# SonyResearch/micro_diffusion

Measured on NVIDIA H100. Metric: training images/sec (global batch 2048), higher is better.
Workload: dtype bf16

## Files before the change

### micro_diffusion_b200/csrc/attn.cu

```cuda
#include <stdlib.h>

#include <initializer_list>

#include "common.cuh"

namespace md {

constexpr int kTile = 64;

__device__ __forceinline__ void ldsm_x4(uint32_t (&r)[4], const void* p) {
  const uint32_t a = static_cast<uint32_t>(__cvta_generic_to_shared(p));
  asm volatile("ldmatrix.sync.aligned.m8n8.x4.shared.b16 {%0,%1,%2,%3}, [%4];"
               : "=r"(r[0]), "=r"(r[1]), "=r"(r[2]), "=r"(r[3])
               : "r"(a));
}
__device__ __forceinline__ void ldsm_x4_t(uint32_t (&r)[4], const void* p) {
  const uint32_t a = static_cast<uint32_t>(__cvta_generic_to_shared(p));
  asm volatile("ldmatrix.sync.aligned.m8n8.x4.trans.shared.b16 {%0,%1,%2,%3}, [%4];"
               : "=r"(r[0]), "=r"(r[1]), "=r"(r[2]), "=r"(r[3])
               : "r"(a));
}
__device__ __forceinline__ void mma16816(float (&d)[4], const uint32_t (&a)[4], uint32_t b0, uint32_t b1) {
  asm volatile(
      "mma.sync.aligned.m16n8k16.row.col.f32.bf16.bf16.f32 {%0,%1,%2,%3}, {%4,%5,%6,%7}, {%8,%9}, {%0,%1,%2,%3};"
// ... 303 lines not shown
  if constexpr (!kFragsInSmem) {
    load_a_frags<HD>(ka, sk, warp * 16, lane);
    load_a_frags<HD>(va, sv, warp * 16, lane);
  }

  float dkacc[HD / 8][4], dvacc[HD / 8][4];
#pragma unroll
  for (int i = 0; i < HD / 8; ++i)
#pragma unroll
    for (int j = 0; j < 4; ++j) dkacc[i][j] = dvacc[i][j] = 0.f;

  for (int q0 = 0, it = 0; q0 < Tq; q0 += kTile, ++it) {
    const __nv_bfloat16* sq = sqdo + (it & 1) * (2 * kTile * P);
    const __nv_bfloat16* sdo = sq + kTile * P;
    const float* slse = sstat + (it & 1) * 2 * kTile;
    const float* sdelta = slse + kTile;
    if (q0 + kTile < Tq) {
      prefetch(q0 + kTile, (it + 1) & 1);
      cp_async_wait<1>();
    } else {
      cp_async_wait<0>();
    }
    __syncthreads();
    float st[8][4], dpt[8][4];
#pragma unroll
    for (int i = 0; i < 8; ++i)
#pragma unroll
      for (int j = 0; j < 4; ++j) st[i][j] = dpt[i][j] = 0.f;
    if constexpr (kFragsInSmem) {
      mma_sa_bt<HD>(st, sk, warp * 16, sq, lane);
      mma_sa_bt<HD>(dpt, sv, warp * 16, sdo, lane);
    } else {
      mma_a_bt<HD>(st, ka, sq, lane);
      mma_a_bt<HD>(dpt, va, sdo, lane);
    }
#pragma unroll
    for (int nt = 0; nt < 8; ++nt)
#pragma unroll
      for (int j = 0; j < 4; ++j) {
        const int qc = nt * 8 + 2 * t + (j & 1);
        const float p = exp2f(st[nt][j] * scale_log2 - slse[qc]);
        st[nt][j] = p;
        dpt[nt][j] = p * (dpt[nt][j] - sdelta[qc]);
      }
    uint32_t pa[4][4];
    acc_to_afrag(pa, st);
    mma_p_m<HD>(dvacc, pa, sdo, lane);
    acc_to_afrag(pa, dpt);
    mma_p_m<HD>(dkacc, pa, sq, lane);
    __syncthreads();
  }
#pragma unroll
  for (int r = 0; r < 2; ++r) {
    const int key = k0 + warp * 16 + g + r * 8;
    if (key < Tk) {
      __nv_bfloat16* pk = dk + (b * Tk + key) * lddk + h * HD;
      __nv_bfloat16* pv = dv + (b * Tk + key) * lddv + h * HD;
#pragma unroll
      for (int i = 0; i < HD / 8; ++i) {
        *reinterpret_cast<uint32_t*>(pk + i * 8 + 2 * t) = pack2(dkacc[i][2 * r] * scale, dkacc[i][2 * r + 1] * scale);
        *reinterpret_cast<uint32_t*>(pv + i * 8 + 2 * t) = pack2(dvacc[i][2 * r], dvacc[i][2 * r + 1]);
      }
    }
  }
}

template <int HD>
__global__ void __launch_bounds__(128)
attn_bwd_dq_kernel(const __nv_bfloat16* __restrict__ dout, long long lddo, const __nv_bfloat16* __restrict__ q,
                   long long ldq, const __nv_bfloat16* __restrict__ k, long long ldk,
                   const __nv_bfloat16* __restrict__ v, long long ldv, const float* __restrict__ lse,
                   const float* __restrict__ delta, __nv_bfloat16* __restrict__ dq, long long lddq, int H, int Tq,
                   int Tk, float scale, float scale_log2) {
  constexpr int P = Smem<HD>::kPitch;
  __shared__ __align__(16) __nv_bfloat16 sq[kTile * P];
  __shared__ __align__(16) __nv_bfloat16 sdo[kTile * P];
  extern __shared__ __align__(16) unsigned char smem_dq[];
  __nv_bfloat16* skv = reinterpret_cast<__nv_bfloat16*>(smem_dq);
  const int warp = threadIdx.x >> 5, lane = threadIdx.x & 31;
  const int g = lane >> 2, t = lane & 3;
  const int h = blockIdx.y;
  const long long b = blockIdx.z;
  const int q0 = blockIdx.x * kTile;
  const __nv_bfloat16* kg = k + b * Tk * ldk;
  const __nv_bfloat16* vg = v + b * Tk * ldv;

  load_tile_async<HD>(skv, kg, ldk, 0, Tk, h * HD);
  load_tile_async<HD>(skv + kTile * P, vg, ldv, 0, Tk, h * HD);
  cp_async_commit();
  load_tile<HD>(sq, q + b * Tq * ldq, ldq, q0, Tq, h * HD);
  load_tile<HD>(sdo, dout + b * Tq * lddo, lddo, q0, Tq, h * HD);
  __syncthreads();
  uint32_t qa[HD / 16][4], doa[HD / 16][4];
  load_a_frags<HD>(qa, sq, warp * 16, lane);
  load_a_frags<HD>(doa, sdo, warp * 16, lane);
  float lrow[2], drow[2];
#pragma unroll
  for (int r = 0; r < 2; ++r) {
    const int row = q0 + warp * 16 + g + r * 8;
    lrow[r] = row < Tq ? lse[(b * H + h) * Tq + row] : INFINITY;
    drow[r] = row < Tq ? delta[(b * H + h) * Tq + row] : 0.f;
  }
  float dqacc[HD / 8][4];
#pragma unroll
  for (int i = 0; i < HD / 8; ++i)
#pragma unroll
    for (int j = 0; j < 4; ++j) dqacc[i][j] = 0.f;

  for (int k0 = 0, it = 0; k0 < Tk; k0 += kTile, ++it) {
    __nv_bfloat16* sk = skv + (it & 1) * (2 * kTile * P);
    __nv_bfloat16* sv = sk + kTile * P;
    if (k0 + kTile < Tk) {
      __nv_bfloat16* nk = skv + ((it + 1) & 1) * (2 * kTile * P);
      load_tile_async<HD>(nk, kg, ldk, k0 + kTile, Tk, h * HD);
      load_tile_async<HD>(nk + kTile * P, vg, ldv, k0 + kTile, Tk, h * HD);
      cp_async_commit();
      cp_async_wait<1>();
    } else {
      cp_async_wait<0>();
    }
    __syncthreads();
    float s[8][4], dp[8][4];
#pragma unroll
    for (int i = 0; i < 8; ++i)
#pragma unroll
      for (int j = 0; j < 4; ++j) s[i][j] = dp[i][j] = 0.f;
    mma_a_bt<HD>(s, qa, sk, lane);
    mma_a_bt<HD>(dp, doa, sv, lane);
#pragma unroll
    for (int nt = 0; nt < 8; ++nt)
#pragma unroll
      for (int j = 0; j < 4; ++j) {
        const int key = k0 + nt * 8 + 2 * t + (j & 1);
        const float p = key < Tk ? exp2f(s[nt][j] * scale_log2 - lrow[j >> 1]) : 0.f;
        s[nt][j] = p * (dp[nt][j] - drow[j >> 1]);
      }
    uint32_t pa[4][4];
    acc_to_afrag(pa, s);
    mma_p_m<HD>(dqacc, pa, sk, lane);
    __syncthreads();
  }
#pragma unroll
  for (int r = 0; r < 2; ++r) {
    const int row = q0 + warp * 16 + g + r * 8;
    if (row < Tq) {
      __nv_bfloat16* dst = dq + (b * Tq + row) * lddq + h * HD;
#pragma unroll
      for (int i = 0; i < HD / 8; ++i)
        *reinterpret_cast<uint32_t*>(dst + i * 8 + 2 * t) = pack2(dqacc[i][2 * r] * scale, dqacc[i][2 * r + 1] * scale);
    }
  }
}

template <int HD, int KT>
__global__ void __launch_bounds__(128)
attn_bwd_small_kernel(const __nv_bfloat16* __restrict__ dout, long long lddo, const __nv_bfloat16* __restrict__ q,
                      long long ldq, const __nv_bfloat16* __restrict__ k, long long ldk,
                      const __nv_bfloat16* __restrict__ v, long long ldv, const float* __restrict__ lse,
                      __nv_bfloat16* __restrict__ dq, long long lddq, __nv_bfloat16* __restrict__ dk, long long lddk,
                      __nv_bfloat16* __restrict__ dv, long long lddv, int H, int Tq, int Tk, float scale,
                      float scale_log2) {
  constexpr int P = Smem<HD>::kPitch;
  constexpr int PP = KT + 8;
  extern __shared__ __align__(16) unsigned char smem_small[];
  __nv_bfloat16* sq = reinterpret_cast<__nv_bfloat16*>(smem_small);
  __nv_bfloat16* sdo = sq + kTile * P;
  __nv_bfloat16* sk = sdo + kTile * P;
  __nv_bfloat16* sv = sk + KT * P;
  static_assert(kTile * (KT + 8) <= KT * Smem<HD>::kPitch || HD == 32, "P copy must fit in the K tile");
  __nv_bfloat16* sp = (HD == 64) ? sk : sv + KT * P;
  __nv_bfloat16* sds = (HD == 64) ? sv : sp + kTile * PP;
  const int warp = threadIdx.x >> 5, lane = threadIdx.x & 31;
  const int g = lane >> 2, t = lane & 3;
  const int h = blockIdx.x;
  const long long b = blockIdx.y;

  load_tile<HD>(sq, q + b * Tq * ldq, ldq, 0, Tq, h * HD);
  load_tile<HD>(sdo, dout + b * Tq * lddo, lddo, 0, Tq, h * HD);
  load_tile<HD, KT>(sk, k + b * Tk * ldk, ldk, 0, Tk, h * HD);
  load_tile<HD, KT>(sv, v + b * Tk * ldv, ldv, 0, Tk, h * HD);
  float lrow[2];
#pragma unroll
  for (int r = 0; r < 2; ++r) {
    const int row = warp * 16 + g + r * 8;
    lrow[r] = row < Tq ? lse[(b * H + h) * Tq + row] : INFINITY;
  }
  __syncthreads();

  uint32_t qa[HD / 16][4], doa[HD / 16][4];
  load_a_frags<HD>(qa, sq, warp * 16, lane);
  load_a_frags<HD>(doa, sdo, warp * 16, lane);
  float s[KT / 8][4], dp[KT / 8][4];
#pragma unroll
  for (int i = 0; i < KT / 8; ++i)
#pragma unroll
    for (int j = 0; j < 4; ++j) s[i][j] = dp[i][j] = 0.f;
  mma_a_bt<HD, KT>(s, qa, sk, lane);
  mma_a_bt<HD, KT>(dp, doa, sv, lane);
  float dsum[2] = {0.f, 0.f};
#pragma unroll
  for (int nt = 0; nt < KT / 8; ++nt)
#pragma unroll
    for (int j = 0; j < 4; ++j) {
      const int key = nt * 8 + 2 * t + (j & 1);
      const float p = key < Tk ? exp2f(s[nt][j] * scale_log2 - lrow[j >> 1]) : 0.f;
      s[nt][j] = p;
      dsum[j >> 1] += p * dp[nt][j];
    }
#pragma unroll
  for (int r = 0; r < 2; ++r) {
    dsum[r] += __shfl_xor_sync(0xffffffffu, dsum[r], 1);
    dsum[r] += __shfl_xor_sync(0xffffffffu, dsum[r], 2);
  }
#pragma unroll
  for (int nt = 0; nt < KT / 8; ++nt)
#pragma unroll
    for (int j = 0; j < 4; ++j) dp[nt][j] = s[nt][j] * (dp[nt][j] - dsum[j >> 1]);
  {
    uint32_t pa[KT / 16][4];
    acc_to_afrag<KT / 16>(pa, dp);
    float dqacc[HD / 8][4];
#pragma unroll
    for (int i = 0; i < HD / 8; ++i)
#pragma unroll
      for (int j = 0; j < 4; ++j) dqacc[i][j] = 0.f;
    mma_p_m<HD, KT>(dqacc, pa, sk, lane);
#pragma unroll
    for (int r = 0; r < 2; ++r) {
      const int row = warp * 16 + g + r * 8;
      if (row < Tq) {
        __nv_bfloat16* dst = dq + (b * Tq + row) * lddq + h * HD;
#pragma unroll
        for (int i = 0; i < HD / 8; ++i)
          *reinterpret_cast<uint32_t*>(dst + i * 8 + 2 * t) = pack2(dqacc[i][2 * r] * scale, dqacc[i][2 * r + 1] * scale);
      }
    }
  }
  __syncthreads();
#pragma unroll
  for (int nt = 0; nt < KT / 8; ++nt)
#pragma unroll
    for (int r = 0; r < 2; ++r) {
      const int row = warp * 16 + g + r * 8;
      *reinterpret_cast<uint32_t*>(sp + row * PP + nt * 8 + 2 * t) = pack2(s[nt][2 * r], s[nt][2 * r + 1]);
      *reinterpret_cast<uint32_t*>(sds + row * PP + nt * 8 + 2 * t) = pack2(dp[nt][2 * r], dp[nt][2 * r + 1]);
    }
  __syncthreads();
  for (int kb = warp; kb < KT / 16; kb += 4) {
    uint32_t pta[4][4], dsta[4][4];
#pragma unroll
    for (int ks = 0; ks < 4; ++ks) {
      const int mi = lane >> 3;
      const int rowq = ks * 16 + (lane & 7) + (mi >> 1) * 8;
      const int colk = kb * 16 + (mi & 1) * 8;
      ldsm_x4_t(pta[ks], sp + rowq * PP + colk);
      ldsm_x4_t(dsta[ks], sds + rowq * PP + colk);
    }
    float dvacc[HD / 8][4], dkacc[HD / 8][4];
#pragma unroll
    for (int i = 0; i < HD / 8; ++i)
#pragma unroll
      for (int j = 0; j < 4; ++j) dvacc[i][j] = dkacc[i][j] = 0.f;
    mma_p_m<HD, 64>(dvacc, pta, sdo, lane);
    mma_p_m<HD, 64>(dkacc, dsta, sq, lane);
#pragma unroll
    for (int r = 0; r < 2; ++r) {
      const int key = kb * 16 + g + r * 8;
      if (key < Tk) {
        __nv_bfloat16* pk = dk + (b * Tk + key) * lddk + h * HD;
        __nv_bfloat16* pv = dv + (b * Tk + key) * lddv + h * HD;
#pragma unroll
        for (int i = 0; i < HD / 8; ++i) {
          *reinterpret_cast<uint32_t*>(pk + i * 8 + 2 * t) = pack2(dkacc[i][2 * r] * scale, dkacc[i][2 * r + 1] * scale);
          *reinterpret_cast<uint32_t*>(pv + i * 8 + 2 * t) = pack2(dvacc[i][2 * r], dvacc[i][2 * r + 1]);
        }
      }
    }
  }
}

template <int HD, int DP>
__device__ __forceinline__ void mma_p_m_slice(float (&out)[2][4], const uint32_t (&pa)[4][4], const __nv_bfloat16* m,
                                              int lane, int dp) {
#pragma unroll
  for (int kt = 0; kt < 4; ++kt) {
    uint32_t b[4];
    const int mi = lane >> 3;
    ldsm_x4_t(b, m + (kt * 16 + (lane & 7) + (mi & 1) * 8) * Smem<HD>::kPitch + dp * 16 + (mi >> 1) * 8);
    mma16816(out[0], pa[kt], b[0], b[1]);
    mma16816(out[1], pa[kt], b[2], b[3]);
  }
}

template <int HD, int KT>
__global__ void __launch_bounds__(128)
attn_bwd_cross_kernel(const __nv_bfloat16* __restrict__ dout, long long lddo, const __nv_bfloat16* __restrict__ q,
                      long long ldq, const __nv_bfloat16* __restrict__ k, long long ldk,
                      const __nv_bfloat16* __restrict__ v, long long ldv, const float* __restrict__ lse,
                      __nv_bfloat16* __restrict__ dq, long long lddq, __nv_bfloat16* __restrict__ dk, long long lddk,
                      __nv_bfloat16* __restrict__ dv, long long lddv, int H, int Tq, int Tk, float scale,
                      float scale_log2) {
  constexpr int P = Smem<HD>::kPitch;
  constexpr int PP = KT + 8;
  constexpr bool kExtra = KT > 64;
  constexpr int kSliceWarps = HD / 16;
  extern __shared__ __align__(16) unsigned char smem_cross[];
  __nv_bfloat16* sk = reinterpret_cast<__nv_bfloat16*>(smem_cross);
  __nv_bfloat16* sv = sk + KT * P;
  __nv_bfloat16* sqdo = sv + KT * P;
  __nv_bfloat16* sp = sqdo + 4 * kTile * P;
  __nv_bfloat16* sds = sp + kTile * PP;
  const int warp = threadIdx.x >> 5, lane = threadIdx.x & 31;
  const int g = lane >> 2, t = lane & 3;
  const int h = blockIdx.x;
  const long long b = blockIdx.y;
  const __nv_bfloat16* qg = q + b * Tq * ldq;
  const __nv_bfloat16* dog = dout + b * Tq * lddo;
  const float* lseg = lse + (b * H + h) * Tq;

  auto prefetch = [&](int q0, int buf) {
    __nv_bfloat16* dst = sqdo + buf * (2 * kTile * P);
    load_tile_async<HD>(dst, qg, ldq, q0, Tq, h * HD);
    load_tile_async<HD>(dst + kTile * P, dog, lddo, q0, Tq, h * HD);
    cp_async_commit();
  };
  load_tile_async<HD, KT>(sk, k + b * Tk * ldk, ldk, 0, Tk, h * HD);
  load_tile_async<HD, KT>(sv, v + b * Tk * ldv, ldv, 0, Tk, h * HD);
  prefetch(0, 0);

  float dvacc[HD / 8][4], dkacc[HD / 8][4];
  float dvx[2][4], dkx[2][4];
#pragma unroll
  for (int i = 0; i < HD / 8; ++i)
#pragma unroll
    for (int j = 0; j < 4; ++j) dvacc[i][j] = dkacc[i][j] = 0.f;
#pragma unroll
  for (int i = 0; i < 2; ++i)
#pragma unroll
    for (int j = 0; j < 4; ++j) dvx[i][j] = dkx[i][j] = 0.f;

  for (int q0 = 0, it = 0; q0 < Tq; q0 += kTile, ++it) {
    const __nv_bfloat16* sq = sqdo + (it & 1) * (2 * kTile * P);
    const __nv_bfloat16* sdo = sq + kTile * P;
    float lrow[2];
#pragma unroll
    for (int r = 0; r < 2; ++r) {
      const int row = q0 + warp * 16 + g + r * 8;
      lrow[r] = row < Tq ? lseg[row] : INFINITY;
    }
    if (q0 + kTile < Tq) {
      prefetch(q0 + kTile, (it + 1) & 1);
      cp_async_wait<1>();
    } else {
      cp_async_wait<0>();
    }
    __syncthreads();

    uint32_t qa[HD / 16][4], doa[HD / 16][4];
    load_a_frags<HD>(qa, sq, warp * 16, lane);
    load_a_frags<HD>(doa, sdo, warp * 16, lane);
    float s[KT / 8][4], dp[KT / 8][4];
#pragma unroll
    for (int i = 0; i < KT / 8; ++i)
#pragma unroll
      for (int j = 0; j < 4; ++j) s[i][j] = dp[i][j] = 0.f;
    mma_a_bt<HD, KT>(s, qa, sk, lane);
    mma_a_bt<HD, KT>(dp, doa, sv, lane);
    float dsum[2] = {0.f, 0.f};
#pragma unroll
    for (int nt = 0; nt < KT / 8; ++nt)
#pragma unroll
      for (int j = 0; j < 4; ++j) {
        const int key = nt * 8 + 2 * t + (j & 1);
        const float pr = key < Tk ? exp2f(s[nt][j] * scale_log2 - lrow[j >> 1]) : 0.f;
        s[nt][j] = pr;
        dsum[j >> 1] += pr * dp[nt][j];
      }
#pragma unroll
    for (int r = 0; r < 2; ++r) {
      dsum[r] += __shfl_xor_sync(0xffffffffu, dsum[r], 1);
      dsum[r] += __shfl_xor_sync(0xffffffffu, dsum[r], 2);
    }
#pragma unroll
    for (int nt = 0; nt < KT / 8; ++nt)
#pragma unroll
      for (int j = 0; j < 4; ++j) dp[nt][j] = s[nt][j] * (dp[nt][j] - dsum[j >> 1]);
    {
      uint32_t pa[KT / 16][4];
      acc_to_afrag<KT / 16>(pa, dp);
      float dqacc[HD / 8][4];
#pragma unroll
      for (int i = 0; i < HD / 8; ++i)
#pragma unroll
        for (int j = 0; j < 4; ++j) dqacc[i][j] = 0.f;
      mma_p_m<HD, KT>(dqacc, pa, sk, lane);
#pragma unroll
      for (int r = 0; r < 2; ++r) {
        const int row = q0 + warp * 16 + g + r * 8;
        if (row < Tq) {
          __nv_bfloat16* dst = dq + (b * Tq + row) * lddq + h * HD;
#pragma unroll
          for (int i = 0; i < HD / 8; ++i)
            *reinterpret_cast<uint32_t*>(dst + i * 8 + 2 * t) = pack2(dqacc[i][2 * r] * scale, dqacc[i][2 * r + 1] * scale);
        }
      }
    }
#pragma unroll
    for (int nt = 0; nt < KT / 8; ++nt)
#pragma unroll
      for (int r = 0; r < 2; ++r) {
        const int row = warp * 16 + g + r * 8;
        *reinterpret_cast<uint32_t*>(sp + row * PP + nt * 8 + 2 * t) = pack2(s[nt][2 * r], s[nt][2 * r + 1]);
        *reinterpret_cast<uint32_t*>(sds + row * PP + nt * 8 + 2 * t) = pack2(dp[nt][2 * r], dp[nt][2 * r + 1]);
      }
    __syncthreads();
    {
      uint32_t pta[4][4], dsta[4][4];
#pragma unroll
      for (int ks = 0; ks < 4; ++ks) {
        const int mi = lane >> 3;
        const int rowq = ks * 16 + (lane & 7) + (mi >> 1) * 8;
        const int colk = warp * 16 + (mi & 1) * 8;
        ldsm_x4_t(pta[ks], sp + rowq * PP + colk);
        ldsm_x4_t(dsta[ks], sds + rowq * PP + colk);
      }
      mma_p_m<HD, 64>(dvacc, pta, sdo, lane);
      mma_p_m<HD, 64>(dkacc, dsta, sq, lane);
      if (kExtra && warp < kSliceWarps) {
#pragma unroll
        for (int ks = 0; ks < 4; ++ks) {
          const int mi = lane >> 3;
          const int rowq = ks * 16 + (lane & 7) + (mi >> 1) * 8;
          const int colk = 64 + (mi & 1) * 8;
          ldsm_x4_t(pta[ks], sp + rowq * PP + colk);
          ldsm_x4_t(dsta[ks], sds + rowq * PP + colk);
        }
        mma_p_m_slice<HD, 0>(dvx, pta, sdo, lane, warp);
        mma_p_m_slice<HD, 0>(dkx, dsta, sq, lane, warp);
      }
    }
    __syncthreads();
  }

#pragma unroll
  for (int r = 0; r < 2; ++r) {
// ... 230 lines not shown
```

### micro_diffusion_b200/csrc/attn_wgmma.cu

```cuda
#include <cuda.h>

#include "common.cuh"
#include "ptx.cuh"
#include "tensormap.cuh"

namespace md {
namespace attn_wg {

constexpr int kHd = 64;
constexpr int kQ = 64;
constexpr int kMaxKeys = 256;
constexpr int kOffK = kQ * kHd * 2;
constexpr int kOffV = kOffK + kMaxKeys * kHd * 2;
constexpr int kOffBar = kOffV + kMaxKeys * kHd * 2;
constexpr int kSmemBytes = kOffBar + 64 + 1024;

__device__ __forceinline__ float ex2_approx(float x) {
  float y;
  asm("ex2.approx.ftz.f32 %0, %1;" : "=f"(y) : "f"(x));
  return y;
}
__device__ __forceinline__ uint32_t pack2(float a, float b) {
  __nv_bfloat162 v = __floats2bfloat162_rn(a, b);
  return *reinterpret_cast<uint32_t*>(&v);
// ... 194 lines not shown
    }
    wgmma_commit();
    wgmma_wait<0>();
    wgmma_fence_operands(s);

    float mx[2] = {-INFINITY, -INFINITY};
#pragma unroll
    for (int j = 0; j < 8; ++j)
#pragma unroll
      for (int i = 0; i < 2; ++i)
#pragma unroll
        for (int e = 0; e < 2; ++e) {
          float& v = s[4 * j + 2 * i + e];
          if (c * 64 + 8 * j + cq + e >= Tk) v = -INFINITY;
          mx[i] = fmaxf(mx[i], v);
        }
    float corr[2];
#pragma unroll
    for (int i = 0; i < 2; ++i) {
      mx[i] = fmaxf(mx[i], __shfl_xor_sync(0xffffffffu, mx[i], 1));
      mx[i] = fmaxf(mx[i], __shfl_xor_sync(0xffffffffu, mx[i], 2));
      const float mn = fmaxf(m2[i], mx[i] * sl2);
      corr[i] = ex2_approx(m2[i] - mn);
      m2[i] = mn;
      l[i] *= corr[i];
    }
#pragma unroll
    for (int j = 0; j < 8; ++j)
#pragma unroll
      for (int i = 0; i < 2; ++i)
#pragma unroll
        for (int e = 0; e < 2; ++e) {
          float& v = s[4 * j + 2 * i + e];
          v = ex2_approx(fmaf(v, sl2, -m2[i]));
          l[i] += v;
        }
#pragma unroll
    for (int x = 0; x < 2; ++x)
#pragma unroll
      for (int j = 0; j < 8; ++j)
#pragma unroll
        for (int i = 0; i < 2; ++i) {
          oacc[x][4 * j + 2 * i] *= corr[i];
          oacc[x][4 * j + 2 * i + 1] *= corr[i];
        }

    uint32_t pa[4][4];
#pragma unroll
    for (int t = 0; t < 4; ++t)
#pragma unroll
      for (int r = 0; r < 4; ++r) pa[t][r] = pack2(s[8 * t + 2 * r], s[8 * t + 2 * r + 1]);
    const uint64_t dv0 = wgmma_smem_desc(smem_u32(st + 2 * kBox), 64 * 128, 1024);
    const uint64_t dv1 = wgmma_smem_desc(smem_u32(st + 3 * kBox), 64 * 128, 1024);
    wgmma_fence();
#pragma unroll
    for (int t = 0; t < 4; ++t) {
      wgmma_m64n64k16_rs<1>(oacc[0], pa[t], dv0 + static_cast<uint64_t>(t * 128), 1u);
      wgmma_m64n64k16_rs<1>(oacc[1], pa[t], dv1 + static_cast<uint64_t>(t * 128), 1u);
    }
    wgmma_commit();
    wgmma_wait<0>();
    wgmma_fence_operands(oacc[0]);
    wgmma_fence_operands(oacc[1]);
    __syncthreads();
    if (threadIdx.x == 0 && c + 2 < nc) load_chunk(c + 2);
  }

#pragma unroll
  for (int i = 0; i < 2; ++i) {
    l[i] += __shfl_xor_sync(0xffffffffu, l[i], 1);
    l[i] += __shfl_xor_sync(0xffffffffu, l[i], 2);
  }
#pragma unroll
  for (int i = 0; i < 2; ++i) {
    const int row = qb * kQ + warp * 16 + (lane >> 2) + 8 * i;
    if (row < Tq) {
      const float inv = __fdividef(1.f, l[i]);
      __nv_bfloat16* dst = o + (static_cast<long long>(b) * Tq + row) * ldo + col0 + cq;
#pragma unroll
      for (int x = 0; x < 2; ++x)
#pragma unroll
        for (int j = 0; j < 8; ++j)
          *reinterpret_cast<uint32_t*>(dst + 64 * x + 8 * j) =
              pack2(oacc[x][4 * j + 2 * i] * inv, oacc[x][4 * j + 2 * i + 1] * inv);
      if ((lane & 3) == 0) lse[(static_cast<long long>(b) * H + h) * Tq + row] = m2[i] + __log2f(l[i]);
    }
  }
}

int make_map(CUtensorMap* map, const void* ptr, long long cols, long long rows, long long batch, long long ld,
             int box_rows) {
  const TmapKey key = make_tmap_key(ptr, cols, rows, batch, ld, rows * ld, 64, box_rows, CU_TENSOR_MAP_SWIZZLE_128B,
                                    CU_TENSOR_MAP_L2_PROMOTION_L2_256B);
  if (cached_tensor_map(map, key) != CUDA_SUCCESS)
    return md_set_error(MD_ERR_CUDA, "attention (wgmma): cuTensorMapEncodeTiled failed");
  return 0;
}

}
}

extern "C" int md_attn_fwd_tc(const void* q, int64_t ldq, const void* k, int64_t ldk, const void* v, int64_t ldv, void* o,
                              int64_t ldo, float* lse, int64_t B, int64_t H, int64_t Tq, int64_t Tk, int64_t hd,
                              void* stream) {
  using namespace md;
  using namespace md::attn_wg;
  if (B <= 0 || H <= 0 || Tq <= 0 || Tk <= 0) return B == 0 ? 0 : md_set_error(MD_ERR_INVALID, "md_attn_fwd_tc: bad sizes");
  if (!(hd == kHd && Tk <= kMaxKeys) && hd != kHd128)
    return md_set_error(MD_ERR_UNSUPPORTED, "md_attn_fwd_tc: needs head_dim 64 with Tk <= 256, or head_dim 128");
  if (!q || !k || !v || !o || !lse) return md_set_error(MD_ERR_INVALID, "md_attn_fwd_tc: null pointer");
  const uintptr_t align = reinterpret_cast<uintptr_t>(q) | reinterpret_cast<uintptr_t>(k) | reinterpret_cast<uintptr_t>(v) |
                          reinterpret_cast<uintptr_t>(o);
  if ((align & 15) != 0 || ((ldq | ldk | ldv | ldo) % 8) != 0)
    return md_set_error(MD_ERR_INVALID, "md_attn_fwd_tc: operands must be 16-byte aligned with pitches % 8 == 0");
  CUtensorMap tmQ, tmK, tmV;
  const dim3 grid(static_cast<unsigned>((Tq + kQ - 1) / kQ), static_cast<unsigned>(H), static_cast<unsigned>(B));
  const float sl2 = 1.4426950408889634f / sqrtf(static_cast<float>(hd));
  if (hd == kHd128) {
    if (int rc = make_map(&tmQ, q, H * hd, Tq, B, ldq, kQ)) return rc;
    if (int rc = make_map(&tmK, k, H * hd, Tk, B, ldk, 64)) return rc;
    if (int rc = make_map(&tmV, v, H * hd, Tk, B, ldv, 64)) return rc;
    static bool attr128 = false;
    if (!attr128) {
      cudaError_t e =
          cudaFuncSetAttribute(attn_fwd_wgmma128_kernel, cudaFuncAttributeMaxDynamicSharedMemorySize, k128SmemBytes);
      if (e != cudaSuccess) return md_set_error(MD_ERR_CUDA, cudaGetErrorString(e));
      attr128 = true;
    }
    attn_fwd_wgmma128_kernel<<<grid, 128, k128SmemBytes, reinterpret_cast<cudaStream_t>(stream)>>>(
        tmQ, tmK, tmV, reinterpret_cast<__nv_bfloat16*>(o), ldo, lse, static_cast<int>(H), static_cast<int>(Tq),
        static_cast<int>(Tk), sl2);
    return check_launch("md_attn_fwd_tc");
  }
  const int kbox = static_cast<int>((Tk + 63) / 64 * 64);
  if (int rc = make_map(&tmQ, q, H * hd, Tq, B, ldq, kQ)) return rc;
  if (int rc = make_map(&tmK, k, H * hd, Tk, B, ldk, kbox)) return rc;
  if (int rc = make_map(&tmV, v, H * hd, Tk, B, ldv, kbox)) return rc;
  static bool attr = false;
  if (!attr) {
    cudaError_t e = cudaFuncSetAttribute(attn_fwd_wgmma_kernel, cudaFuncAttributeMaxDynamicSharedMemorySize, kSmemBytes);
    if (e != cudaSuccess) return md_set_error(MD_ERR_CUDA, cudaGetErrorString(e));
    attr = true;
  }
  attn_fwd_wgmma_kernel<<<grid, 128, kSmemBytes, reinterpret_cast<cudaStream_t>(stream)>>>(
      tmQ, tmK, tmV, reinterpret_cast<__nv_bfloat16*>(o), ldo, lse, static_cast<int>(H), static_cast<int>(Tq),
      static_cast<int>(Tk), sl2);
  return check_launch("md_attn_fwd_tc");
}

namespace md {
namespace attn_wg {

constexpr int kTileBytes = 64 * kHd * 2;
constexpr int kBwdSmemBytes = 4 * kTileBytes + 64 + 1024;

__device__ __forceinline__ void to_a_frags(const float (&acc)[32], uint32_t (&a)[4][4]) {
#pragma unroll
  for (int t = 0; t < 4; ++t)
#pragma unroll
    for (int r = 0; r < 4; ++r) a[t][r] = pack2(acc[8 * t + 2 * r], acc[8 * t + 2 * r + 1]);
}

__device__ __forceinline__ void mm_nt(float (&c)[32], const uint8_t* x, const uint8_t* y) {
  const uint64_t dx = wgmma_smem_desc(smem_u32(x), 16, 1024), dy = wgmma_smem_desc(smem_u32(y), 16, 1024);
#pragma unroll
  for (int k = 0; k < kHd / 16; ++k) wgmma_m64n64k16<0, 0>(c, dx + 2 * k, dy + 2 * k, k > 0 ? 1u : 0u);
}
__device__ __forceinline__ void mm_rs(float (&c)[32], const uint32_t (&a)[4][4], const uint8_t* y) {
  const uint64_t dy = wgmma_smem_desc(smem_u32(y), 64 * 128, 1024);
#pragma unroll
  for (int t = 0; t < 4; ++t) wgmma_m64n64k16_rs<1>(c, a[t], dy + static_cast<uint64_t>(t * 128), 1u);
}

__global__ void __launch_bounds__(128)
attn_bwd_wgmma_kernel(const __grid_constant__ CUtensorMap tmQ, const __grid_constant__ CUtensorMap tmK,
                      const __grid_constant__ CUtensorMap tmV, const __grid_constant__ CUtensorMap tmdO,
                      const float* __restrict__ lse, const float* __restrict__ delta, __nv_bfloat16* __restrict__ dq,
                      long long lddq, __nv_bfloat16* __restrict__ dk, long long lddk, __nv_bfloat16* __restrict__ dv,
                      long long lddv, int H, int Tq, int Tk, float scale, float sl2, int kv_blocks) {
  extern __shared__ uint8_t smem_raw[];
  uint8_t* smem = reinterpret_cast<uint8_t*>((reinterpret_cast<uintptr_t>(smem_raw) + 1023) & ~static_cast<uintptr_t>(1023));
  uint64_t* bar = reinterpret_cast<uint64_t*>(smem + 4 * kTileBytes);
  uint8_t* f0 = smem;
  uint8_t* f1 = smem + kTileBytes;
  uint8_t* s0 = smem + 2 * kTileBytes;
  uint8_t* s1 = smem + 3 * kTileBytes;
  const bool kv_role = static_cast<int>(blockIdx.x) < kv_blocks;
  const int blk = kv_role ? blockIdx.x : blockIdx.x - kv_blocks;
  const int h = blockIdx.y, b = blockIdx.z;
  const int warp = threadIdx.x >> 5, lane = threadIdx.x & 31;
  const int cq = 2 * (lane & 3);
  const int r0 = warp * 16 + (lane >> 2);
  const long long stat0 = (static_cast<long long>(b) * H + h) * Tq;
  const int n_iter = kv_role ? (Tq + 63) / 64 : (Tk + 63) / 64;

  if (threadIdx.x == 0) {
    tma_prefetch_desc(&tmQ); tma_prefetch_desc(&tmK); tma_prefetch_desc(&tmV); tma_prefetch_desc(&tmdO);
    mbar_init(bar, 1);
    mbar_fence_init();
  }
  __syncthreads();
  float acc0[32], acc1[32];
#pragma unroll
  for (int i = 0; i < 32; ++i) acc0[i] = acc1[i] = 0.f;

  for (int it = 0; it < n_iter; ++it) {
    if (threadIdx.x == 0) {
      if (it == 0) {
        mbar_expect_tx(bar, 4 * kTileBytes);
        if (kv_role) {
          tma_load_3d(&tmK, bar, f0, h * kHd, blk * 64, b);
          tma_load_3d(&tmV, bar, f1, h * kHd, blk * 64, b);
        } else {
          tma_load_3d(&tmQ, bar, f0, h * kHd, blk * 64, b);
          tma_load_3d(&tmdO, bar, f1, h * kHd, blk * 64, b);
        }
      } else {
        mbar_expect_tx(bar, 2 * kTileBytes);
      }
      if (kv_role) {
        tma_load_3d(&tmQ, bar, s0, h * kHd, it * 64, b);
        tma_load_3d(&tmdO, bar, s1, h * kHd, it * 64, b);
      } else {
        tma_load_3d(&tmK, bar, s0, h * kHd, it * 64, b);
        tma_load_3d(&tmV, bar, s1, h * kHd, it * 64, b);
      }
    }
    mbar_wait(bar, it & 1);

    float sc[32], dp[32];
    wgmma_fence();
    if (kv_role) {
      mm_nt(sc, f0, s0);
      mm_nt(dp, f1, s1);
    } else {
      mm_nt(sc, f0, s0);
      mm_nt(dp, f1, s1);
    }
    wgmma_commit();
    wgmma_wait<0>();
    wgmma_fence_operands(sc);
    wgmma_fence_operands(dp);

#pragma unroll
    for (int i = 0; i < 2; ++i) {
      float lrow = 0.f, drow = 0.f;
      if (!kv_role) {
        const int q = blk * 64 + r0 + 8 * i;
        lrow = q < Tq ? lse[stat0 + q] : INFINITY;
        drow = q < Tq ? delta[stat0 + q] : 0.f;
      }
#pragma unroll
      for (int j = 0; j < 8; ++j)
#pragma unroll
        for (int e = 0; e < 2; ++e) {
          const int col = it * 64 + 8 * j + cq + e;
          float l2, dl;
          bool valid;
          if (kv_role) {
            valid = col < Tq;
            l2 = valid ? lse[stat0 + col] : INFINITY;
            dl = valid ? delta[stat0 + col] : 0.f;
          } else {
            valid = col < Tk;
            l2 = lrow;
            dl = drow;
          }
          const int x = 4 * j + 2 * i + e;
          const float p = valid ? ex2_approx(fmaf(sc[x], sl2, -l2)) : 0.f;
          sc[x] = p;
          dp[x] = p * (dp[x] - dl);
        }
    }
    uint32_t pa[4][4], da[4][4];
    to_a_frags(sc, pa);
    to_a_frags(dp, da);
    wgmma_fence();
    if (kv_role) {
      mm_rs(acc0, pa, s1);
      mm_rs(acc1, da, s0);
    } else {
      mm_rs(acc0, da, s0);
    }
    wgmma_commit();
    wgmma_wait<0>();
    wgmma_fence_operands(acc0);
    wgmma_fence_operands(acc1);
    __syncthreads();
  }

#pragma unroll
  for (int i = 0; i < 2; ++i) {
    const int row = blk * 64 + r0 + 8 * i;
    if (kv_role) {
      if (row < Tk) {
        __nv_bfloat16* pv = dv + (static_cast<long long>(b) * Tk + row) * lddv + h * kHd + cq;
        __nv_bfloat16* pk = dk + (static_cast<long long>(b) * Tk + row) * lddk + h * kHd + cq;
#pragma unroll
        for (int j = 0; j < 8; ++j) {
          *reinterpret_cast<uint32_t*>(pv + 8 * j) = pack2(acc0[4 * j + 2 * i], acc0[4 * j + 2 * i + 1]);
          *reinterpret_cast<uint32_t*>(pk + 8 * j) = pack2(acc1[4 * j + 2 * i] * scale, acc1[4 * j + 2 * i + 1] * scale);
        }
      }
    } else if (row < Tq) {
      __nv_bfloat16* pq = dq + (static_cast<long long>(b) * Tq + row) * lddq + h * kHd + cq;
#pragma unroll
      for (int j = 0; j < 8; ++j)
        *reinterpret_cast<uint32_t*>(pq + 8 * j) = pack2(acc0[4 * j + 2 * i] * scale, acc0[4 * j + 2 * i + 1] * scale);
    }
  }
}

}

int attn_bwd_wgmma(const void* dout, int64_t lddo, const void* q, int64_t ldq, const void* k, int64_t ldk, const void* v,
                   int64_t ldv, const float* lse, const float* delta, void* dq, int64_t lddq, void* dk, int64_t lddk,
                   void* dv, int64_t lddv, int64_t B, int64_t H, int64_t Tq, int64_t Tk, cudaStream_t stream) {
  using namespace attn_wg;
  CUtensorMap tmQ, tmK, tmV, tmdO;
  if (int rc = make_map(&tmQ, q, H * kHd, Tq, B, ldq, 64)) return rc;
  if (int rc = make_map(&tmK, k, H * kHd, Tk, B, ldk, 64)) return rc;
  if (int rc = make_map(&tmV, v, H * kHd, Tk, B, ldv, 64)) return rc;
  if (int rc = make_map(&tmdO, dout, H * kHd, Tq, B, lddo, 64)) return rc;
  static bool attr = false;
  if (!attr) {
    cudaError_t e = cudaFuncSetAttribute(attn_bwd_wgmma_kernel, cudaFuncAttributeMaxDynamicSharedMemorySize, kBwdSmemBytes);
    if (e != cudaSuccess) return md_set_error(MD_ERR_CUDA, cudaGetErrorString(e));
    attr = true;
  }
  const int kv_blocks = static_cast<int>((Tk + 63) / 64), q_blocks = static_cast<int>((Tq + 63) / 64);
  const dim3 grid(static_cast<unsigned>(kv_blocks + q_blocks), static_cast<unsigned>(H), static_cast<unsigned>(B));
  const float scale = 1.f / sqrtf(static_cast<float>(kHd));
  attn_bwd_wgmma_kernel<<<grid, 128, kBwdSmemBytes, stream>>>(
      tmQ, tmK, tmV, tmdO, lse, delta, reinterpret_cast<__nv_bfloat16*>(dq), lddq, reinterpret_cast<__nv_bfloat16*>(dk),
      lddk, reinterpret_cast<__nv_bfloat16*>(dv), lddv, static_cast<int>(H), static_cast<int>(Tq), static_cast<int>(Tk),
      scale, scale * 1.4426950408889634f, kv_blocks);
  return check_launch("md_attn_bwd_tc");
}

}
```

Baseline: 1208.

## Pipeline attention backward with multi-stage TMA ring and split small-kernel work

Replaces the single-buffered wgmma attention backward loop with a 3-stage TMA ring buffer using full/empty mbarriers, and splits the kernel into separate dK/dV and dQ paths. LSE and delta values are staged in shared memory, and two wgmma groups are committed separately so softmax work can overlap the second matmul. The small backward kernel now loads tiles with cp.async and spreads the extra 64-key block across all warps by head-dim slice instead of leaving one warp to do it. This adds more shared memory and more complex barrier logic, which could reduce occupancy.

```diff
diff --git a/micro_diffusion_b200/csrc/attn.cu b/micro_diffusion_b200/csrc/attn.cu
--- a/micro_diffusion_b200/csrc/attn.cu
+++ b/micro_diffusion_b200/csrc/attn.cu
@@ -479,6 +479,19 @@
   }
 }
 
+template <int HD, int DP>
+__device__ __forceinline__ void mma_p_m_slice(float (&out)[2][4], const uint32_t (&pa)[4][4], const __nv_bfloat16* m,
+                                              int lane, int dp) {
+#pragma unroll
+  for (int kt = 0; kt < 4; ++kt) {
+    uint32_t b[4];
+    const int mi = lane >> 3;
+    ldsm_x4_t(b, m + (kt * 16 + (lane & 7) + (mi & 1) * 8) * Smem<HD>::kPitch + dp * 16 + (mi >> 1) * 8);
+    mma16816(out[0], pa[kt], b[0], b[1]);
+    mma16816(out[1], pa[kt], b[2], b[3]);
+  }
+}
+
 template <int HD, int KT>
 __global__ void __launch_bounds__(128)
 attn_bwd_small_kernel(const __nv_bfloat16* __restrict__ dout, long long lddo, const __nv_bfloat16* __restrict__ q,
@@ -502,16 +515,18 @@
   const int h = blockIdx.x;
   const long long b = blockIdx.y;
 
-  load_tile<HD>(sq, q + b * Tq * ldq, ldq, 0, Tq, h * HD);
-  load_tile<HD>(sdo, dout + b * Tq * lddo, lddo, 0, Tq, h * HD);
-  load_tile<HD, KT>(sk, k + b * Tk * ldk, ldk, 0, Tk, h * HD);
-  load_tile<HD, KT>(sv, v + b * Tk * ldv, ldv, 0, Tk, h * HD);
+  load_tile_async<HD>(sq, q + b * Tq * ldq, ldq, 0, Tq, h * HD);
+  load_tile_async<HD>(sdo, dout + b * Tq * lddo, lddo, 0, Tq, h * HD);
+  load_tile_async<HD, KT>(sk, k + b * Tk * ldk, ldk, 0, Tk, h * HD);
+  load_tile_async<HD, KT>(sv, v + b * Tk * ldv, ldv, 0, Tk, h * HD);
+  cp_async_commit();
   float lrow[2];
 #pragma unroll
   for (int r = 0; r < 2; ++r) {
     const int row = warp * 16 + g + r * 8;
     lrow[r] = row < Tq ? lse[(b * H + h) * Tq + row] : INFINITY;
   }
+  cp_async_wait<0>();
   __syncthreads();
 
   uint32_t qa[HD / 16][4], doa[HD / 16][4];
@@ -573,7 +588,8 @@
       *reinterpret_cast<uint32_t*>(sds + row * PP + nt * 8 + 2 * t) = pack2(dp[nt][2 * r], dp[nt][2 * r + 1]);
     }
   __syncthreads();
-  for (int kb = warp; kb < KT / 16; kb += 4) {
+  constexpr bool kSplit = HD == 64 && KT > 64;
+  for (int kb = warp; kb < (kSplit ? 4 : KT / 16); kb += 4) {
     uint32_t pta[4][4], dsta[4][4];
 #pragma unroll
     for (int ks = 0; ks < 4; ++ks) {
@@ -604,20 +620,39 @@
       }
     }
   }
-}
-
-template <int HD, int DP>
-__device__ __forceinline__ void mma_p_m_slice(float (&out)[2][4], const uint32_t (&pa)[4][4], const __nv_bfloat16* m,
-                                              int lane, int dp) {
-#pragma unroll
-  for (int kt = 0; kt < 4; ++kt) {
-    uint32_t b[4];
-    const int mi = lane >> 3;
-    ldsm_x4_t(b, m + (kt * 16 + (lane & 7) + (mi & 1) * 8) * Smem<HD>::kPitch + dp * 16 + (mi >> 1) * 8);
-    mma16816(out[0], pa[kt], b[0], b[1]);
-    mma16816(out[1], pa[kt], b[2], b[3]);
-  }
-}
+  if constexpr (kSplit) {
+    uint32_t pta[4][4], dsta[4][4];
+#pragma unroll
+    for (int ks = 0; ks < 4; ++ks) {
+      const int mi = lane >> 3;
+      const int rowq = ks * 16 + (lane & 7) + (mi >> 1) * 8;
+      const int colk = 64 + (mi & 1) * 8;
+      ldsm_x4_t(pta[ks], sp + rowq * PP + colk);
+      ldsm_x4_t(dsta[ks], sds + rowq * PP + colk);
+    }
+    float dvx[2][4], dkx[2][4];
+#pragma unroll
+    for (int i = 0; i < 2; ++i)
+#pragma unroll
+      for (int j = 0; j < 4; ++j) dvx[i][j] = dkx[i][j] = 0.f;
+    mma_p_m_slice<HD, 0>(dvx, pta, sdo, lane, warp);
+    mma_p_m_slice<HD, 0>(dkx, dsta, sq, lane, warp);
+#pragma unroll
+    for (int r = 0; r < 2; ++r) {
+      const int key = 64 + g + r * 8;
+      if (key < Tk) {
+        __nv_bfloat16* pk = dk + (b * Tk + key) * lddk + h * HD + warp * 16;
+        __nv_bfloat16* pv = dv + (b * Tk + key) * lddv + h * HD + warp * 16;
+#pragma unroll
+        for (int i = 0; i < 2; ++i) {
+          *reinterpret_cast<uint32_t*>(pk + i * 8 + 2 * t) = pack2(dkx[i][2 * r] * scale, dkx[i][2 * r + 1] * scale);
+          *reinterpret_cast<uint32_t*>(pv + i * 8 + 2 * t) = pack2(dvx[i][2 * r], dvx[i][2 * r + 1]);
+        }
+      }
+    }
+  }
+}
+
 
 template <int HD, int KT>
 __global__ void __launch_bounds__(128)
diff --git a/micro_diffusion_b200/csrc/attn_wgmma.cu b/micro_diffusion_b200/csrc/attn_wgmma.cu
--- a/micro_diffusion_b200/csrc/attn_wgmma.cu
+++ b/micro_diffusion_b200/csrc/attn_wgmma.cu
@@ -370,7 +370,11 @@
 namespace attn_wg {
 
 constexpr int kTileBytes = 64 * kHd * 2;
-constexpr int kBwdSmemBytes = 4 * kTileBytes + 64 + 1024;
+constexpr int kBwdStages = 3;
+constexpr int kOffRing = 2 * kTileBytes;
+constexpr int kOffStat = kOffRing + kBwdStages * 2 * kTileBytes;
+constexpr int kOffBwdBar = kOffStat + kBwdStages * 128 * 4;
+constexpr int kBwdSmemBytes = kOffBwdBar + 2 * kBwdStages * 8 + 1024;
 
 __device__ __forceinline__ void to_a_frags(const float (&acc)[32], uint32_t (&a)[4][4]) {
 #pragma unroll
@@ -388,6 +392,230 @@
   const uint64_t dy = wgmma_smem_desc(smem_u32(y), 64 * 128, 1024);
 #pragma unroll
   for (int t = 0; t < 4; ++t) wgmma_m64n64k16_rs<1>(c, a[t], dy + static_cast<uint64_t>(t * 128), 1u);
+}
+
+struct BwdArgs {
+  const float* lse;
+  const float* delta;
+  __nv_bfloat16* dq;
+  long long lddq;
+  __nv_bfloat16* dk;
+  long long lddk;
+  __nv_bfloat16* dv;
+  long long lddv;
+  int H, Tq, Tk;
+  float scale, sl2;
+};
+
+__device__ __forceinline__ void bwd_load(const CUtensorMap* fa, const CUtensorMap* fb, const CUtensorMap* sa,
+                                         const CUtensorMap* sb, uint8_t* smem, uint64_t* full, int fixed_row, int n,
+                                         int col, int b) {
+  const int s = n % kBwdStages;
+  uint8_t* st = smem + kOffRing + s * 2 * kTileBytes;
+  mbar_expect_tx(&full[s], (n == 0 ? 4 : 2) * kTileBytes);
+  if (n == 0) {
+    tma_load_3d(fa, &full[0], smem, col, fixed_row, b);
+    tma_load_3d(fb, &full[0], smem + kTileBytes, col, fixed_row, b);
+  }
+  tma_load_3d(sa, &full[s], st, col, n * 64, b);
+  tma_load_3d(sb, &full[s], st + kTileBytes, col, n * 64, b);
+}
+
+__device__ __forceinline__ void bwd_dkdv(const CUtensorMap* tmQ, const CUtensorMap* tmK, const CUtensorMap* tmV,
+                                         const CUtensorMap* tmdO, uint8_t* smem, uint64_t* full, uint64_t* empty,
+                                         const BwdArgs& a, int blk, int h, int b) {
+  const int t = threadIdx.x, warp = t >> 5, lane = t & 31;
+  const int cq = 2 * (lane & 3);
+  const int r0 = warp * 16 + (lane >> 2);
+  const long long stat0 = (static_cast<long long>(b) * a.H + h) * a.Tq;
+  float* stat = reinterpret_cast<float*>(smem + kOffStat);
+  const int n_iter = (a.Tq + 63) / 64;
+  auto load_stat = [&](int n) -> float {
+    const int q = n * 64 + (t & 63);
+    if (t < 64) return q < a.Tq ? a.lse[stat0 + q] : INFINITY;
+    return q < a.Tq ? a.delta[stat0 + q] : 0.f;
+  };
+  if (t == 0)
+    for (int n = 0; n < kBwdStages && n < n_iter; ++n) bwd_load(tmK, tmV, tmQ, tmdO, smem, full, blk * 64, n, h * kHd, b);
+  float first_stat[kBwdStages];
+#pragma unroll
+  for (int n = 0; n < kBwdStages; ++n) first_stat[n] = n < n_iter ? load_stat(n) : 0.f;
+#pragma unroll
+  for (int n = 0; n < kBwdStages; ++n) {
+    if (n < n_iter) {
+      stat[n * 128 + t] = first_stat[n];
+      mbar_arrive(&full[n]);
+    }
+  }
+
+  float dvacc[32], dkacc[32];
+#pragma unroll
+  for (int i = 0; i < 32; ++i) dvacc[i] = dkacc[i] = 0.f;
+  for (int it = 0; it < n_iter; ++it) {
+    const int s = it % kBwdStages;
+    const uint32_t par = (it / kBwdStages) & 1;
+    const uint8_t* sQ = smem + kOffRing + s * 2 * kTileBytes;
+    const uint8_t* sdO = sQ + kTileBytes;
+    const float* sl = stat + s * 128;
+    const bool refill = it + kBwdStages < n_iter;
+    const float next_stat = refill ? load_stat(it + kBwdStages) : 0.f;
+    mbar_wait(&full[s], par);
+
+    float sc[32], dp[32];
+    wgmma_fence();
+    mm_nt(sc, smem, sQ);
+    wgmma_commit();
+    mm_nt(dp, smem + kTileBytes, sdO);
+    wgmma_commit();
+    wgmma_wait<1>();
+    wgmma_fence_operands(sc);
+#pragma unroll
+    for (int j = 0; j < 8; ++j)
+#pragma unroll
+      for (int e = 0; e < 2; ++e) {
+        const int col = 8 * j + cq + e;
+        const bool valid = it * 64 + col < a.Tq;
+        const float l2 = sl[col];
+#pragma unroll
+        for (int i = 0; i < 2; ++i) {
+          float& x = sc[4 * j + 2 * i + e];
+          x = valid ? ex2_approx(fmaf(x, a.sl2, -l2)) : 0.f;
+        }
+      }
+    uint32_t pa[4][4];
+    to_a_frags(sc, pa);
+    wgmma_fence();
+    mm_rs(dvacc, pa, sdO);
+    wgmma_commit();
+    wgmma_wait<1>();
+    wgmma_fence_operands(dp);
+#pragma unroll
+    for (int j = 0; j < 8; ++j)
+#pragma unroll
+      for (int e = 0; e < 2; ++e) {
+        const float dl = sl[64 + 8 * j + cq + e];
+#pragma unroll
+        for (int i = 0; i < 2; ++i) {
+          const int x = 4 * j + 2 * i + e;
+          dp[x] = sc[x] * (dp[x] - dl);
+        }
+      }
+    uint32_t da[4][4];
+    to_a_frags(dp, da);
+    wgmma_fence();
+    mm_rs(dkacc, da, sQ);
+    wgmma_commit();
+    wgmma_wait<0>();
+    wgmma_fence_operands(dvacc);
+    wgmma_fence_operands(dkacc);
+    if (lane == 0) mbar_arrive(&empty[s]);
+    if (refill) {
+      mbar_wait(&empty[s], par);
+      if (t == 0) bwd_load(tmK, tmV, tmQ, tmdO, smem, full, blk * 64, it + kBwdStages, h * kHd, b);
+      stat[s * 128 + t] = next_stat;
+      mbar_arrive(&full[s]);
+    }
+  }
+
+#pragma unroll
+  for (int i = 0; i < 2; ++i) {
+    const int row = blk * 64 + r0 + 8 * i;
+    if (row < a.Tk) {
+      __nv_bfloat16* pv = a.dv + (static_cast<long long>(b) * a.Tk + row) * a.lddv + h * kHd + cq;
+      __nv_bfloat16* pk = a.dk + (static_cast<long long>(b) * a.Tk + row) * a.lddk + h * kHd + cq;
+#pragma unroll
+      for (int j = 0; j < 8; ++j) {
+        *reinterpret_cast<uint32_t*>(pv + 8 * j) = pack2(dvacc[4 * j + 2 * i], dvacc[4 * j + 2 * i + 1]);
+        *reinterpret_cast<uint32_t*>(pk + 8 * j) =
+            pack2(dkacc[4 * j + 2 * i] * a.scale, dkacc[4 * j + 2 * i + 1] * a.scale);
+      }
+    }
+  }
+}
+
+__device__ __forceinline__ void bwd_dq(const CUtensorMap* tmQ, const CUtensorMap* tmK, const CUtensorMap* tmV,
+                                       const CUtensorMap* tmdO, uint8_t* smem, uint64_t* full, uint64_t* empty,
+                                       const BwdArgs& a, int blk, int h, int b) {
+  const int t = threadIdx.x, warp = t >> 5, lane = t & 31;
+  const int cq = 2 * (lane & 3);
+  const int r0 = warp * 16 + (lane >> 2);
+  const long long stat0 = (static_cast<long long>(b) * a.H + h) * a.Tq;
+  const int n_iter = (a.Tk + 63) / 64;
+  if (t == 0)
+    for (int n = 0; n < kBwdStages && n < n_iter; ++n) bwd_load(tmQ, tmdO, tmK, tmV, smem, full, blk * 64, n, h * kHd, b);
+  float lrow[2], drow[2];
+#pragma unroll
+  for (int i = 0; i < 2; ++i) {
+    const int q = blk * 64 + r0 + 8 * i;
+    lrow[i] = q < a.Tq ? a.lse[stat0 + q] : INFINITY;
+    drow[i] = q < a.Tq ? a.delta[stat0 + q] : 0.f;
+  }
+
+  float dqacc[32];
+#pragma unroll
+  for (int i = 0; i < 32; ++i) dqacc[i] = 0.f;
+  for (int it = 0; it < n_iter; ++it) {
+    const int s = it % kBwdStages;
+    const uint32_t par = (it / kBwdStages) & 1;
+    const uint8_t* sK = smem + kOffRing + s * 2 * kTileBytes;
+    const uint8_t* sV = sK + kTileBytes;
+    mbar_wait(&full[s], par);
+
+    float sc[32], dp[32];
+    wgmma_fence();
+    mm_nt(sc, smem, sK);
+    wgmma_commit();
+    mm_nt(dp, smem + kTileBytes, sV);
+    wgmma_commit();
+    wgmma_wait<1>();
+    wgmma_fence_operands(sc);
+#pragma unroll
+    for (int j = 0; j < 8; ++j)
+#pragma unroll
+      for (int e = 0; e < 2; ++e) {
+        const bool valid = it * 64 + 8 * j + cq + e < a.Tk;
+#pragma unroll
+        for (int i = 0; i < 2; ++i) {
+          float& x = sc[4 * j + 2 * i + e];
+          x = valid ? ex2_approx(fmaf(x, a.sl2, -lrow[i])) : 0.f;
+        }
+      }
+    wgmma_wait<0>();
+    wgmma_fence_operands(dp);
+#pragma unroll
+    for (int j = 0; j < 8; ++j)
+#pragma unroll
+      for (int e = 0; e < 2; ++e)
+#pragma unroll
+        for (int i = 0; i < 2; ++i) {
+          const int x = 4 * j + 2 * i + e;
+          dp[x] = sc[x] * (dp[x] - drow[i]);
+        }
+    uint32_t da[4][4];
+    to_a_frags(dp, da);
+    wgmma_fence();
+    mm_rs(dqacc, da, sK);
+    wgmma_commit();
+    wgmma_wait<0>();
+    wgmma_fence_operands(dqacc);
+    if (lane == 0) mbar_arrive(&empty[s]);
+    if (t == 0 && it + kBwdStages < n_iter) {
+      mbar_wait(&empty[s], par);
+      bwd_load(tmQ, tmdO, tmK, tmV, smem, full, blk * 64, it + kBwdStages, h * kHd, b);
+    }
+  }
+
+#pragma unroll
+  for (int i = 0; i < 2; ++i) {
+    const int row = blk * 64 + r0 + 8 * i;
+    if (row < a.Tq) {
+      __nv_bfloat16* pq = a.dq + (static_cast<long long>(b) * a.Tq + row) * a.lddq + h * kHd + cq;
+#pragma unroll
+      for (int j = 0; j < 8; ++j)
+        *reinterpret_cast<uint32_t*>(pq + 8 * j) =
+            pack2(dqacc[4 * j + 2 * i] * a.scale, dqacc[4 * j + 2 * i + 1] * a.scale);
+    }
+  }
 }
 
 __global__ void __launch_bounds__(128)
@@ -398,135 +626,21 @@
                       long long lddv, int H, int Tq, int Tk, float scale, float sl2, int kv_blocks) {
   extern __shared__ uint8_t smem_raw[];
   uint8_t* smem = reinterpret_cast<uint8_t*>((reinterpret_cast<uintptr_t>(smem_raw) + 1023) & ~static_cast<uintptr_t>(1023));
-  uint64_t* bar = reinterpret_cast<uint64_t*>(smem + 4 * kTileBytes);
-  uint8_t* f0 = smem;
-  uint8_t* f1 = smem + kTileBytes;
-  uint8_t* s0 = smem + 2 * kTileBytes;
-  uint8_t* s1 = smem + 3 * kTileBytes;
+  uint64_t* full = reinterpret_cast<uint64_t*>(smem + kOffBwdBar);
+  uint64_t* empty = full + kBwdStages;
   const bool kv_role = static_cast<int>(blockIdx.x) < kv_blocks;
-  const int blk = kv_role ? blockIdx.x : blockIdx.x - kv_blocks;
-  const int h = blockIdx.y, b = blockIdx.z;
-  const int warp = threadIdx.x >> 5, lane = threadIdx.x & 31;
-  const int cq = 2 * (lane & 3);
-  const int r0 = warp * 16 + (lane >> 2);
-  const long long stat0 = (static_cast<long long>(b) * H + h) * Tq;
-  const int n_iter = kv_role ? (Tq + 63) / 64 : (Tk + 63) / 64;
-
   if (threadIdx.x == 0) {
     tma_prefetch_desc(&tmQ); tma_prefetch_desc(&tmK); tma_prefetch_desc(&tmV); tma_prefetch_desc(&tmdO);
-    mbar_init(bar, 1);
+    for (int s = 0; s < kBwdStages; ++s) {
+      mbar_init(&full[s], kv_role ? 1 + 128 : 1);
+      mbar_init(&empty[s], 4);
+    }
     mbar_fence_init();
   }
   __syncthreads();
-  float acc0[32], acc1[32];
-#pragma unroll
-  for (int i = 0; i < 32; ++i) acc0[i] = acc1[i] = 0.f;
-
-  for (int it = 0; it < n_iter; ++it) {
-    if (threadIdx.x == 0) {
-      if (it == 0) {
-        mbar_expect_tx(bar, 4 * kTileBytes);
-        if (kv_role) {
-          tma_load_3d(&tmK, bar, f0, h * kHd, blk * 64, b);
-          tma_load_3d(&tmV, bar, f1, h * kHd, blk * 64, b);
-        } else {
-          tma_load_3d(&tmQ, bar, f0, h * kHd, blk * 64, b);
-          tma_load_3d(&tmdO, bar, f1, h * kHd, blk * 64, b);
-        }
-      } else {
-        mbar_expect_tx(bar, 2 * kTileBytes);
-      }
-      if (kv_role) {
-        tma_load_3d(&tmQ, bar, s0, h * kHd, it * 64, b);
-        tma_load_3d(&tmdO, bar, s1, h * kHd, it * 64, b);
-      } else {
-        tma_load_3d(&tmK, bar, s0, h * kHd, it * 64, b);
-        tma_load_3d(&tmV, bar, s1, h * kHd, it * 64, b);
-      }
-    }
-    mbar_wait(bar, it & 1);
-
-    float sc[32], dp[32];
-    wgmma_fence();
-    if (kv_role) {
-      mm_nt(sc, f0, s0);
-      mm_nt(dp, f1, s1);
-    } else {
-      mm_nt(sc, f0, s0);
-      mm_nt(dp, f1, s1);
-    }
-    wgmma_commit();
-    wgmma_wait<0>();
-    wgmma_fence_operands(sc);
-    wgmma_fence_operands(dp);
-
-#pragma unroll
-    for (int i = 0; i < 2; ++i) {
-      float lrow = 0.f, drow = 0.f;
-      if (!kv_role) {
-        const int q = blk * 64 + r0 + 8 * i;
-        lrow = q < Tq ? lse[stat0 + q] : INFINITY;
-        drow = q < Tq ? delta[stat0 + q] : 0.f;
-      }
-#pragma unroll
-      for (int j = 0; j < 8; ++j)
-#pragma unroll
-        for (int e = 0; e < 2; ++e) {
-          const int col = it * 64 + 8 * j + cq + e;
-          float l2, dl;
-          bool valid;
-          if (kv_role) {
-            valid = col < Tq;
-            l2 = valid ? lse[stat0 + col] : INFINITY;
-            dl = valid ? delta[stat0 + col] : 0.f;
-          } else {
-            valid = col < Tk;
-            l2 = lrow;
-            dl = drow;
-          }
-          const int x = 4 * j + 2 * i + e;
-          const float p = valid ? ex2_approx(fmaf(sc[x], sl2, -l2)) : 0.f;
-          sc[x] = p;
-          dp[x] = p * (dp[x] - dl);
-        }
-    }
-    uint32_t pa[4][4], da[4][4];
-    to_a_frags(sc, pa);
-    to_a_frags(dp, da);
-    wgmma_fence();
-    if (kv_role) {
-      mm_rs(acc0, pa, s1);
-      mm_rs(acc1, da, s0);
-    } else {
-      mm_rs(acc0, da, s0);
-    }
-    wgmma_commit();
-    wgmma_wait<0>();
-    wgmma_fence_operands(acc0);
-    wgmma_fence_operands(acc1);
-    __syncthreads();
-  }
-
-#pragma unroll
-  for (int i = 0; i < 2; ++i) {
-    const int row = blk * 64 + r0 + 8 * i;
-    if (kv_role) {
-      if (row < Tk) {
-        __nv_bfloat16* pv = dv + (static_cast<long long>(b) * Tk + row) * lddv + h * kHd + cq;
-        __nv_bfloat16* pk = dk + (static_cast<long long>(b) * Tk + row) * lddk + h * kHd + cq;
-#pragma unroll
-        for (int j = 0; j < 8; ++j) {
-          *reinterpret_cast<uint32_t*>(pv + 8 * j) = pack2(acc0[4 * j + 2 * i], acc0[4 * j + 2 * i + 1]);
-          *reinterpret_cast<uint32_t*>(pk + 8 * j) = pack2(acc1[4 * j + 2 * i] * scale, acc1[4 * j + 2 * i + 1] * scale);
-        }
-      }
-    } else if (row < Tq) {
-      __nv_bfloat16* pq = dq + (static_cast<long long>(b) * Tq + row) * lddq + h * kHd + cq;
-#pragma unroll
-      for (int j = 0; j < 8; ++j)
-        *reinterpret_cast<uint32_t*>(pq + 8 * j) = pack2(acc0[4 * j + 2 * i] * scale, acc0[4 * j + 2 * i + 1] * scale);
-    }
-  }
+  const BwdArgs a{lse, delta, dq, lddq, dk, lddk, dv, lddv, H, Tq, Tk, scale, sl2};
+  if (kv_role) bwd_dkdv(&tmQ, &tmK, &tmV, &tmdO, smem, full, empty, a, blockIdx.x, blockIdx.y, blockIdx.z);
+  else bwd_dq(&tmQ, &tmK, &tmV, &tmdO, smem, full, empty, a, blockIdx.x - kv_blocks, blockIdx.y, blockIdx.z);
 }
 
 }
```

Measured after the change: 1227, median of 6. 1.6% higher.
